# mmsyan/GoPairingBasedCryptography

Measured on AMD Instinct MI355X. Metric: BN254 pairings/s at batch 2^20 per GPU (+ G1/G2 scalar-mults/s at the same batch in roofline.scalar_mul), higher is better.
Workload: dtype int64; 1 GPU; configs[1]: batch of 1048576 independent bn254.Pair on random (G1,G2) points per GPU; batch_per_gpu=1048576

## Files before the change

### gopairingbasedcryptography_amd/csrc/bn254_constants29.hip.hpp

```cpp
#ifndef GPBC_BN254_CONSTANTS29_HIP_HPP
#define GPBC_BN254_CONSTANTS29_HIP_HPP
#define F29_P {0x187cfd47, 0x010460b6, 0x1c72a34f, 0x02d522d0, 0x1585d978, 0x02db40c0, 0x00a6e141, 0x0e5c2634, 0x0030644e}
#define F29_PINV 0x04866389
#define F29_ONE {0x157ccc21, 0x141c2758, 0x185230d3, 0x014c0419, 0x0aa36fb9, 0x1d4240ce, 0x11d54c07, 0x052ac7a8, 0x000dc836}
#define F29_TO_INTERNAL {0x13349ca1, 0x1a5d84a8, 0x0a3e5cac, 0x100249e0, 0x12b951e8, 0x0e92d304, 0x14cb95b3, 0x041b9d3d, 0x00058003}
#define F29_FROM_INTERNAL {0x058f0d9d, 0x1aea1c6e, 0x11c2cf74, 0x11d651eb, 0x1462c0a7, 0x11b7bc3c, 0x1cbd99ba, 0x183340fb, 0x000e0a77}
#define F29_B_G2 {{0x0b489658, 0x00cfd255, 0x0fdb9a77, 0x02ce89f7, 0x0033a0d4, 0x1a768545, 0x06ee3ddc, 0x106a7dc1, 0x0019316b}, {0x1b9fece0, 0x07ecccd1, 0x1069f1c7, 0x0cdf64f3, 0x0154cbe1, 0x0dd22ac0, 0x06eba4e8, 0x1929a235, 0x00283739}}
#define F29_ISO_T2 {0x130d623a, 0x0ea9efb1, 0x0fb12793, 0x1bf1335a, 0x150f3208, 0x004ff90c, 0x1b07aa3d, 0x1ae371b9, 0x001ff864}
#define F29_ISO_T3 {0x1af1f8a3, 0x00cd9858, 0x1dce6a34, 0x142e620a, 0x1bc0c667, 0x0ae94d20, 0x0db9310b, 0x12572b72, 0x000405e6}
#define F29_ISO_KFIX {0x0629460e, 0x19d018e1, 0x128d20c1, 0x106197be, 0x1858c34e, 0x0e37413a, 0x1c8aaa40, 0x058dc596, 0x0003f1e8}
#define F29_B_G1 {0x00766463, 0x1c54760a, 0x08f6927a, 0x03e40c4d, 0x1fea4f2b, 0x17c6c26a, 0x157fe417, 0x0f8056f9, 0x002958a2}
#define F29_PLAIN_TO_INTERNAL {0x059bac10, 0x0d1503a3, 0x018016b8, 0x10ab0ca8, 0x02632639, 0x02c0169f, 0x169bfd53, 0x11869d4c, 0x002a11a6}
#define F29_PLAIN_ONE {0x00000001, 0x00000000, 0x00000000, 0x00000000, 0x00000000, 0x00000000, 0x00000000, 0x00000000, 0x00000000}
#define F29_HALF_P {0x0c3e7ea3, 0x1082305b, 0x0e3951a7, 0x016a9168, 0x0ac2ecbc, 0x116da060, 0x005370a0, 0x072e131a, 0x00183227}
#define F29_EXP_SQRT {0x161f3f52, 0x1841182d, 0x071ca8d3, 0x00b548b4, 0x0561765e, 0x08b6d030, 0x0029b850, 0x1397098d, 0x000c1913}
#define F29_EXP_P34 {0x161f3f51, 0x1841182d, 0x071ca8d3, 0x00b548b4, 0x0561765e, 0x08b6d030, 0x0029b850, 0x1397098d, 0x000c1913}
#define F29_EXP_P12 {0x0c3e7ea3, 0x1082305b, 0x0e3951a7, 0x016a9168, 0x0ac2ecbc, 0x116da060, 0x005370a0, 0x072e131a, 0x00183227}
#define SVDW_G1_Z {0x157ccc21, 0x141c2758, 0x185230d3, 0x014c0419, 0x0aa36fb9, 0x1d4240ce, 0x11d54c07, 0x052ac7a8, 0x000dc836}
#define SVDW_G1_C1 {0x1d76333d, 0x0f6c3cab, 0x04d61fff, 0x025aed96, 0x1507e56c, 0x122dc278, 0x06ae4ede, 0x064ef86e, 0x0006bc8a}
#define SVDW_G1_C2 {0x01801893, 0x16741caf, 0x1210393d, 0x10c48f5b, 0x057134df, 0x12cc7ff9, 0x1768ca9c, 0x0498af45, 0x00114e0c}
#define SVDW_G1_C3 {0x1b4a814f, 0x1d686287, 0x16a42cba, 0x0bac1e79, 0x013fb16c, 0x1d850693, 0x1eba05b6, 0x0c9dae1e, 0x001b5818}
#define SVDW_G1_C4 {0x068a0e4b, 0x171eba7c, 0x0b55234f, 0x150690b3, 0x0ed0a792, 0x1ff392ca, 0x026922c2, 0x109d85a1, 0x002768eb}
#define SVDW_G2_Z {{0x157ccc21, 0x141c2758, 0x185230d3, 0x014c0419, 0x0aa36fb9, 0x1d4240ce, 0x11d54c07, 0x052ac7a8, 0x000dc836}, {0x00000000, 0x00000000, 0x00000000, 0x00000000, 0x00000000, 0x00000000, 0x00000000, 0x00000000, 0x00000000}}
#define SVDW_G2_C1 {{0x00c56279, 0x14ebf9ae, 0x082dcb4a, 0x041a8e11, 0x0ad7108d, 0x17b8c613, 0x18c389e4, 0x15954569, 0x0026f9a1}, {0x1b9fece0, 0x07ecccd1, 0x1069f1c7, 0x0cdf64f3, 0x0154cbe1, 0x0dd22ac0, 0x06eba4e8, 0x1929a235, 0x00283739}}
#define SVDW_G2_C2 {{0x01801893, 0x16741caf, 0x1210393d, 0x10c48f5b, 0x057134df, 0x12cc7ff9, 0x1768ca9c, 0x0498af45, 0x00114e0c}, {0x00000000, 0x00000000, 0x00000000, 0x00000000, 0x00000000, 0x00000000, 0x00000000, 0x00000000, 0x00000000}}
#define SVDW_G2_C3 {{0x1ac12654, 0x18b51d52, 0x02b71328, 0x0f302745, 0x18dae6df, 0x1ec740f3, 0x0ad8391f, 0x1e701b16, 0x002bf9c5}, {0x1b8c55e3, 0x07029597, 0x09a398b3, 0x06a5295f, 0x152a0cd2, 0x1080d518, 0x1295607f, 0x1129d51a, 0x00151beb}}
#define SVDW_G2_C4 {{0x1a9d7742, 0x1b78c9da, 0x18a8378f, 0x1586dd8a, 0x1c979cde, 0x1b6acebc, 0x159e5ffb, 0x15469a85, 0x002cd11a}, {0x017a140e, 0x0ccd05ab, 0x0dad5994, 0x148069b2, 0x09454dc3, 0x089e4881, 0x1813914c, 0x05d61ecb, 0x002b29a5}}
#define F29_KP_ROWS { \
{50510080, 463423804, 224178423, 182267676, 438732777, 79642451, 421445353, 64605178, -811880051, 0, 0, 0}, \
{461354567, 480487922, 164582470, 229790189, 262955361, 127565844, 432381994, 305525294, -808708645, 0, 0, 0}, \
{335328142, 497552041, 104986517, 277312702, 87177945, 175489237, 443318635, 9574498, -805537238, 0, 0, 0}, \
{209301717, 514616160, 45390564, 324835215, 448271441, 223412629, 454255276, 250494614, -802365832, 0, 0, 0}, \
{83275292, 531680279, 522665523, 372357727, 272494025, 271336022, 465191917, 491414730, -799194426, 0, 0, 0}, \
{494119779, 11873485, 463069571, 419880240, 96716609, 319259415, 476128558, 195463934, -796023019, 0, 0, 0}, \
{368093354, 28937604, 403473618, 467402753, 457810105, 367182807, 487065199, 436384050, -792851613, 0, 0, 0}, \
{242066929, 46001723, 343877665, 514925266, 282032689, 415106200, 498001840, 140433254, -789680206, 0, 0, 0}, \
{116040504, 63065842, 284281712, 25576867, 106255274, 463029593, 508938481, 381353370, -786508800, 0, 0, 0}, \
{526884991, 80129960, 224685759, 73099380, 467348770, 510952985, 519875122, 85402574, -783337393, 0, 0, 0}, \
{400858566, 97194079, 165089806, 120621893, 291571354, 22005466, 530811764, 326322690, -780165987, 0, 0, 0}, \
{274832141, 114258198, 105493853, 168144406, 115793938, 69928859, 4877493, 30371895, -776994580, 0, 0, 0}, \
{148805716, 131322317, 45897900, 215666919, 476887434, 117852251, 15814134, 271292011, -773823174, 0, 0, 0}, \
{22779291, 148386436, 523172859, 263189431, 301110018, 165775644, 26750775, 512212127, -770651768, 0, 0, 0}, \
{433623778, 165450554, 463576906, 310711944, 125332602, 213699037, 37687416, 216261331, -767480361, 0, 0, 0}, \
// ... 545 lines not shown
```

### gopairingbasedcryptography_amd/csrc/gpbc_pairing.hip

```cpp
#include "gpbc_common.hpp"
#include "wide29.hip.hpp"
#include "pairing29.hip.hpp"
#include "pairing29_pair.hip.hpp"

static_assert(LINE_BYTES_PER_PAIR == (size_t)MILLER_LINES * LINE_WORDS * sizeof(int32_t), "lines workspace row size");

__device__ __forceinline__ void line_store(int32_t *__restrict__ buf, size_t stride, size_t lane, int step, const LineS &l) {
    int32_t *b = buf + (size_t)step * LINE_WORDS * stride + lane;
    const Fe *fe[6] = {&l.c0.a0, &l.c0.a1, &l.c3.a0, &l.c3.a1, &l.c4.a0, &l.c4.a1};
#pragma unroll
    for (int e = 0; e < 6; e++)
#pragma unroll
        for (int i = 0; i < NL; i++) b[(size_t)(e * NL + i) * stride] = fe[e]->v[i];
}
__device__ __forceinline__ LineS line_load(const int32_t *__restrict__ buf, size_t stride, size_t lane, int step) {
    const int32_t *b = buf + (size_t)step * LINE_WORDS * stride + lane;
    LineS l;
    Fe *fe[6] = {&l.c0.a0, &l.c0.a1, &l.c3.a0, &l.c3.a1, &l.c4.a0, &l.c4.a1};
#pragma unroll
    for (int e = 0; e < 6; e++)
#pragma unroll
        for (int i = 0; i < NL; i++) fe[e]->v[i] = b[(size_t)(e * NL + i) * stride];
    return l;
}

__shared__ int32_t g_line_stage[27][BLOCK];
__device__ __forceinline__ void line_request(const int32_t *__restrict__ buf, size_t stride, size_t lane, int step, bool odd) {
    const int32_t *b = buf + ((size_t)step * LINE_WORDS + (odd ? 27 : 0)) * stride + lane;
#pragma unroll
    for (int r = 0; r < 27; r++) __builtin_amdgcn_global_load_lds(b + (size_t)r * stride, &g_line_stage[r][0], 4, 0, 0);
}
__device__ __forceinline__ LineS line_from_stage() {
    __builtin_amdgcn_s_waitcnt(0x0F70);
    const unsigned e = threadIdx.x & ~1u;
    LineS l;
    Fe *fe[6] = {&l.c0.a0, &l.c0.a1, &l.c3.a0, &l.c3.a1, &l.c4.a0, &l.c4.a1};
#pragma unroll
    for (int w = 0; w < LINE_WORDS; w++) fe[w / NL]->v[w % NL] = g_line_stage[w < 27 ? w : w - 27][e + (w < 27 ? 0 : 1)];
    __builtin_amdgcn_s_waitcnt(0xC07F);
    return l;
}

GPBC_KERNEL k_miller_lines(const uint8_t *__restrict__ P, const uint8_t *__restrict__ Q, int32_t *__restrict__ lines, size_t n, size_t stride) {
    size_t i = (size_t)blockIdx.x * BLOCK + threadIdx.x;
    if (i >= n) return;
    const uint8_t *p = P + i * GPBC_G1_BYTES, *q = Q + i * GPBC_G2_BYTES;
    if (g1_bytes_inf(p) || g2_bytes_inf(q)) return;
    G1A a{fe_load(p), fe_load(p + 32)};
    G2A b{f2_load(q), f2_load(q + 64)};
    int step = 0;
    miller_lines(a, b, [&](const LineS &l) { line_store(lines, stride, i, step++, l); });
}

GPBC_KERNEL k_miller_accumulate(const uint8_t *__restrict__ P, const uint8_t *__restrict__ Q, const int32_t *__restrict__ lines,
                                uint8_t *__restrict__ f_out, size_t n, size_t stride) {
    size_t lane = (size_t)blockIdx.x * BLOCK + threadIdx.x;
    size_t i = lane >> 1;
    if (i >= n) return;
    PairDpp x{(bool)(lane & 1)};
    const uint8_t *p = P + i * GPBC_G1_BYTES, *q = Q + i * GPBC_G2_BYTES;
    F6 h;
    if (g1_bytes_inf(p) || g2_bytes_inf(q)) h = f12p_one(x);
    else {
        int step = 0;
        line_request(lines, stride, i, 0, x.odd);
        h = miller_accumulate_pair(x, [&]() -> LineS {
            LineS l = line_from_stage();
            if (++step < MILLER_LINES) line_request(lines, stride, i, step, x.odd);
            return l;
        });
    }
    f6_store(f_out + i * GPBC_GT_BYTES + (x.odd ? 192 : 0), h);
}

constexpr size_t PIPELINED_MAX_PAIRS = 16384;
constexpr uint32_t PIPELINED_SPIN_LIMIT = 1u << 22;
GPBC_KERNEL k_miller_pipelined(const uint8_t *__restrict__ P, const uint8_t *__restrict__ Q, int32_t *lines, uint32_t *progress,
                               uint8_t *__restrict__ f_out, size_t n, size_t stride, unsigned n_line_blocks, uint32_t spin_limit) {
    if (blockIdx.x < n_line_blocks) {
        size_t i = (size_t)blockIdx.x * BLOCK + threadIdx.x;
        if (i >= n) return;
        const uint8_t *p = P + i * GPBC_G1_BYTES, *q = Q + i * GPBC_G2_BYTES;
        if (g1_bytes_inf(p) || g2_bytes_inf(q)) return;
        G1A a{fe_load(p), fe_load(p + 32)};
        G2A b{f2_load(q), f2_load(q + 64)};
        int step = 0;
        miller_lines(a, b, [&](const LineS &l) {
            line_store(lines, stride, i, step++, l);
            __hip_atomic_store(progress + i, (uint32_t)step, __ATOMIC_RELEASE, __HIP_MEMORY_SCOPE_AGENT);
        });
        return;
    }
    size_t lane = (size_t)(blockIdx.x - n_line_blocks) * BLOCK + threadIdx.x;
    size_t i = lane >> 1;
    if (i >= n) return;
    PairDpp x{(bool)(lane & 1)};
    const uint8_t *p = P + i * GPBC_G1_BYTES, *q = Q + i * GPBC_G2_BYTES;
    F6 h;
    if (g1_bytes_inf(p) || g2_bytes_inf(q)) h = f12p_one(x);
    else {
        int step = 0;
        bool own_lines = false;
        h = miller_accumulate_pair(x, [&]() -> LineS {
            if (!own_lines) {
                uint32_t spins = 0;
                while (__hip_atomic_load(progress + i, __ATOMIC_ACQUIRE, __HIP_MEMORY_SCOPE_AGENT) <= (uint32_t)step) {
                    __builtin_amdgcn_s_sleep(16);
                    if (++spins > spin_limit) { own_lines = true; break; }
                }
                if (own_lines) {
                    G1A a{fe_load(p), fe_load(p + 32)};
                    G2A b{f2_load(q), f2_load(q + 64)};
                    int s2 = 0;
                    miller_lines(a, b, [&](const LineS &l) { line_store(lines, stride, i, s2++, l); });
                    __threadfence();
                }
            }
            return line_load(lines, stride, i, step++);
        });
    }
    f6_store(f_out + i * GPBC_GT_BYTES + (x.odd ? 192 : 0), h);
}

constexpr int MULTI_CHUNK = 8;
constexpr size_t MULTI_GROUP = 65536;
GPBC_KERNEL k_miller_lines_chunks(const uint8_t *__restrict__ P, const uint8_t *__restrict__ Q, int32_t *__restrict__ lines,
                                  const uint64_t *__restrict__ chunk_off, size_t n_chunks, size_t n_slots, uint64_t *__restrict__ seen_lines) {
    size_t t = (size_t)blockIdx.x * BLOCK + threadIdx.x;
    if (t >= n_slots) return;
    const size_t i = t / n_chunks, c = t % n_chunks;
    const uint64_t c_lo = chunk_off[c], c_hi = chunk_off[c + 1];
    if (i == 0) { seen_lines[2 * c] = c_lo; seen_lines[2 * c + 1] = c_hi; }
    const uint64_t pair = c_lo + i;
    if (pair >= c_hi) return;
    const uint8_t *p = P + pair * GPBC_G1_BYTES, *q = Q + pair * GPBC_G2_BYTES;
    if (g1_bytes_inf(p) || g2_bytes_inf(q)) return;
    G1A a{fe_load(p), fe_load(p + 32)};
    G2A b{f2_load(q), f2_load(q + 64)};
    int step = 0;
    miller_lines(a, b, [&](const LineS &l) { line_store(lines, n_slots, t, step++, l); });
}
GPBC_KERNEL k_miller_accumulate_chunks(const uint8_t *__restrict__ P, const uint8_t *__restrict__ Q, const int32_t *__restrict__ lines,
                                       const uint64_t *__restrict__ chunk_off, uint8_t *__restrict__ f_out, size_t n_chunks, size_t n_slots,
                                       const uint64_t *__restrict__ seen_lines, uint64_t *__restrict__ seen) {
    size_t lane = (size_t)blockIdx.x * BLOCK + threadIdx.x;
    size_t c = lane >> 1;
    if (c >= n_chunks) return;
// ... 14 lines not shown
}

constexpr int FIXED_Q_CHUNK = 64;
GPBC_KERNEL k_q_lines(const uint8_t *__restrict__ Q, int32_t *__restrict__ qlines, size_t m) {
    size_t i = (size_t)blockIdx.x * BLOCK + threadIdx.x;
    if (i >= m) return;
    const uint8_t *q = Q + i * GPBC_G2_BYTES;
    if (g2_bytes_inf(q)) return;
    G2A b{f2_load(q), f2_load(q + 64)};
    int step = 0;
    miller_lines_raw(b, [&](const LineE &l) { line_store(qlines, m, i, step++, LineS{l.r0, l.r1, l.r2}); });
}
constexpr int LINE34_WORDS = 4 * NL;
GPBC_KERNEL k_q_lines_scale(const int32_t *__restrict__ qlines, int32_t *__restrict__ q34, size_t m) {
    size_t t = (size_t)blockIdx.x * BLOCK + threadIdx.x;
    if (t >= m * MILLER_LINES) return;
    const size_t i = t % m;
    const int li = (int)(t / m);
    LineS r = line_load(qlines, m, i, li);
    F2 inv = f2_inv(f2_norm(r.c0));
    F2 c3 = f2_mul(f2_norm(r.c3), inv), c4 = f2_mul(f2_norm(r.c4), inv);
    int32_t *o = q34 + (size_t)li * LINE34_WORDS * m + i;
    const Fe *fe[4] = {&c3.a0, &c3.a1, &c4.a0, &c4.a1};
#pragma unroll
    for (int e = 0; e < 4; e++)
#pragma unroll
        for (int w = 0; w < NL; w++) o[(size_t)(e * NL + w) * m] = fe[e]->v[w];
}
constexpr int LINE_POINT_GROUP = 8;
GPBC_KERNEL_G1 k_g1_line_point(const uint8_t *__restrict__ P, int32_t *__restrict__ out, size_t n) {
    const size_t base = ((size_t)blockIdx.x * BLOCK + threadIdx.x) * LINE_POINT_GROUP;
    if (base >= n) return;
    const int cnt = n - base < (size_t)LINE_POINT_GROUP ? (int)(n - base) : LINE_POINT_GROUP;
    fe_batch_inverse<LINE_POINT_GROUP>(cnt, [&](int j) { return fe_load(P + (base + j) * GPBC_G1_BYTES + 32); }, [&](int j, const Fe &yinv) {
        const uint8_t *pb = P + (base + j) * GPBC_G1_BYTES;
        Fe xoy = fe_mul(fe_load(pb), yinv);
        int32_t *o = out + (base + j) * 20;
#pragma unroll
        for (int w = 0; w < NL; w++) { o[w] = xoy.v[w]; o[NL + w] = yinv.v[w]; }
        o[18] = g1_bytes_inf(pb) ? 1 : 0;
        o[19] = 0;
    });
}
GPBC_KERNEL k_miller_accumulate_fixed_q(const int32_t *__restrict__ Pint, const uint8_t *__restrict__ Q, const int32_t *__restrict__ q34,
                                        uint8_t *__restrict__ f_out, size_t m, size_t k, size_t L, size_t n_c) {
    size_t lane = (size_t)blockIdx.x * BLOCK + threadIdx.x;
    size_t t = lane >> 1;
    if (t >= n_c * k) return;
    PairDpp x{(bool)(lane & 1)};
    const size_t c = t / k, j = t % k;
    const size_t lo = c * L, hi = (c + 1) * L < m ? (c + 1) * L : m;
    int vi[FIXED_Q_CHUNK], n = 0;
    for (size_t i = lo; i < hi; i++)
        if (!Pint[(j * m + i) * 20 + 18] && !g2_bytes_inf(Q + i * GPBC_G2_BYTES)) vi[n++] = (int)i;
    F6 h;
    if (n == 0) h = f12p_one(x);
    else h = miller_accumulate_multi_34(x, n, [&](int p, int li) -> Line34 {
        const size_t i = (size_t)vi[p];
        const int32_t *lb = q34 + ((size_t)li * LINE34_WORDS + (x.odd ? 2 * NL : 0)) * m + i;
        const int32_t *pp = Pint + (j * m + i) * 20 + (x.odd ? NL : 0);
        F2 coef;
        Fe pc;
#pragma unroll
        for (int w = 0; w < NL; w++) { coef.a0.v[w] = lb[(size_t)w * m]; coef.a1.v[w] = lb[(size_t)(NL + w) * m]; pc.v[w] = pp[w]; }
        const F2 mine = f2_mul_fe(coef, pc), other = x.swap(mine);
        return Line34{f2_sel(x.odd, other, mine), f2_sel(x.odd, mine, other)};
    });
    f6_store(f_out + (j * n_c + c) * GPBC_GT_BYTES + (x.odd ? 192 : 0), h);
// ... 752 lines not shown
```

### gopairingbasedcryptography_amd/csrc/pairing29.hip.hpp

```cpp
#ifndef GPBC_PAIRING29_HIP_HPP
#define GPBC_PAIRING29_HIP_HPP
#include "bn254_constants.hip.hpp"
#include "tower29.hip.hpp"

namespace gpbc {

struct G1A { Fe x, y; };
struct G2A { F2 x, y; };
struct G2P { F2 x, y, z; };
struct LineE { F2 r0, r1, r2; };

GPBC_INLINE int ate_naf_digit(int i) { constexpr int8_t D[BN254_ATE_NAF_LEN] = BN254_ATE_NAF; return D[i]; }

GPBC_INLINE F2 f2_mul_9mi_n(const F2 &x) {
    return F2{fe_reduce_arith_norm(fe_add(fe_add(fe_mul8_norm(x.a0), x.a0), x.a1)), fe_reduce_arith_norm(fe_sub(fe_add(fe_mul8_norm(x.a1), x.a1), x.a0))};
}
template <bool ISO = false> GPBC_INLINE void g2_double_step(G2P &t, LineE &l) {
    F2 A = f2_halve(f2_mul(t.x, t.y));
    F2 B = f2_sqr(t.y);
    F2 C = f2_sqr(t.z);
    F2 C3 = f2_norm(f2_add(f2_dbl(C), C));
    F2 E = ISO ? f2_mul_9mi_n(C3) : f2_mul(C3, b_twist29());
    F2 F = f2_add(f2_dbl(E), E);
    F2 G = ISO ? f2_add(E, f2_halve(f2_norm(f2_add(B, E)))) : f2_halve(f2_norm(f2_add(B, F)));
// ... 7 lines not shown
    l.r1 = f2_norm(f2_add(f2_dbl(J), J));
    l.r2 = f2_sub(E, B);
}
GPBC_INLINE void g2_add_step(G2P &t, LineE &l, const G2A &q) {
    F2 O = f2_sub(t.y, f2_mul(q.y, t.z));
    F2 L = f2_sub(t.x, f2_mul(q.x, t.z));
    F2 C = f2_sqr(O);
    F2 D = f2_sqr(L);
    F2 E = f2_mul(L, D);
    F2 F = f2_mul(t.z, C);
    F2 G = f2_mul(t.x, D);
    F2 H = f2_norm(f2_sub(f2_add(E, F), f2_dbl(G)));
    F2 t1 = f2_mul(t.y, E);
    t.x = f2_mul(L, H);
    t.y = f2_norm(f2_sub(f2_mul(f2_sub(G, H), O), t1));
    t.z = f2_mul(E, t.z);
    l.r0 = L;
    l.r1 = f2_neg(O);
    l.r2 = f2_sub(f2_mul(q.x, O), f2_mul(L, q.y));
}
GPBC_INLINE void g2_line_step(const G2P &t, LineE &l, const G2A &q) {
    F2 O = f2_sub(t.y, f2_mul(q.y, t.z));
    F2 L = f2_sub(t.x, f2_mul(q.x, t.z));
    l.r0 = L;
    l.r1 = f2_neg(O);
    l.r2 = f2_sub(f2_mul(q.x, O), f2_mul(L, q.y));
}
struct LineS { F2 c0, c3, c4; };
constexpr int MILLER_LINES = 88;
constexpr int LINE_WORDS = 6 * NL;

GPBC_INLINE LineS line_scale(const LineE &l, const G1A &p) { return LineS{f2_mul_fe(l.r0, p.y), f2_mul_fe(l.r1, p.x), l.r2}; }

template <class Sink> GPBC_INLINE void miller_lines(const G1A &p0, const G2A &q0, Sink &&sink) {
    constexpr int32_t T2[NL] = F29_ISO_T2, T3[NL] = F29_ISO_T3, KF[NL] = F29_ISO_KFIX;
    const Fe t2 = fe_const(T2), t3 = fe_const(T3);
    const G1A p{fe_mul(p0.x, t2), fe_mul(p0.y, t3)};
    const G2A q{f2_mul_fe(q0.x, t2), f2_mul_fe(q0.y, t3)};
    G2P t{q.x, q.y, f2_one()};
    const F2 ny = f2_neg(q.y);
    LineE l;
    for (int i = BN254_ATE_NAF_LEN - 2; i >= 0; i--) {
        g2_double_step<true>(t, l);
        sink(line_scale(l, p));
        int d = ate_naf_digit(i);
        if (d != 0) {
            g2_add_step(t, l, G2A{q.x, f2_sel(d > 0, q.y, ny)});
            sink(line_scale(l, p));
        }
    }
    G2A q1{f2_mul(f2_conj(q.x), gamma29(1, 2)), f2_mul(f2_conj(q.y), gamma29(1, 3))};
    G2A q2{f2_mul(q.x, gamma29(2, 2)), f2_neg(f2_mul(q.y, gamma29(2, 3)))};
    g2_add_step(t, l, q1);
    sink(line_scale(l, p));
    g2_line_step(t, l, q2);
    const Fe k = fe_const(KF);
    sink(LineS{f2_mul_fe(l.r0, fe_mul(p.y, k)), f2_mul_fe(l.r1, fe_mul(p.x, k)), f2_mul_fe(l.r2, k)});
}

template <class Sink> GPBC_INLINE void miller_lines_raw(const G2A &q, Sink &&sink) {
    G2P t{q.x, q.y, f2_one()};
    const F2 ny = f2_neg(q.y);
    LineE l;
    for (int i = BN254_ATE_NAF_LEN - 2; i >= 0; i--) {
        g2_double_step(t, l);
        sink(l);
        int d = ate_naf_digit(i);
        if (d != 0) {
            g2_add_step(t, l, G2A{q.x, f2_sel(d > 0, q.y, ny)});
            sink(l);
        }
    }
    G2A q1{f2_mul(f2_conj(q.x), gamma29(1, 2)), f2_mul(f2_conj(q.y), gamma29(1, 3))};
    G2A q2{f2_mul(q.x, gamma29(2, 2)), f2_neg(f2_mul(q.y, gamma29(2, 3)))};
    g2_add_step(t, l, q1);
    sink(l);
    g2_line_step(t, l, q2);
    sink(l);
}

template <int G, class LoadY, class Emit> GPBC_INLINE void fe_batch_inverse(int cnt, LoadY &&y_at, Emit &&emit) {
    Fe y[G], pre[G];
#pragma unroll
    for (int j = 0; j < G; j++) {
        y[j] = fe_one();
        if (j < cnt) {
            Fe v = y_at(j);
            if (!fe_is_zero(v)) y[j] = v;
        }
// ... 117 lines not shown
```

### gopairingbasedcryptography_amd/csrc/pairing29_pair.hip.hpp

```cpp
#ifndef GPBC_PAIRING29_PAIR_HIP_HPP
#define GPBC_PAIRING29_PAIR_HIP_HPP
#include "pairing29.hip.hpp"
#include "tower29_pair.hip.hpp"

namespace gpbc {

template <class X, class Src> GPBC_INLINE F6 miller_accumulate_pair(const X &x, Src &&next) {
    LineS l0 = next();
    F6 h = f6_norm(f6_sel(x.odd, F6{l0.c3, l0.c4, f2_zero()}, F6{l0.c0, f2_zero(), f2_zero()}));
    for (int i = BN254_ATE_NAF_LEN - 2; i >= 0; i--) {
        if (i != BN254_ATE_NAF_LEN - 2) {
            h = f12p_sqr<true>(x, h);
            LineS l = next();
            h = f12p_mul_034<true>(x, h, l.c0, l.c3, l.c4);
        }
        if (ate_naf_digit(i) != 0) {
            LineS l = next();
            h = f12p_mul_034<true>(x, h, l.c0, l.c3, l.c4);
        }
    }
    for (int k = 0; k < 2; k++) {
        LineS l = next();
        h = f12p_mul_034<true>(x, h, l.c0, l.c3, l.c4);
    }
    return h;
}

template <class X, class LineAt> GPBC_INLINE F6 miller_accumulate_multi(const X &x, int m, LineAt &&line) {
    int li = 0;
    auto mul_lines = [&](F6 h, int from) {
        int p = from;
        for (; p + 1 < m; p += 2) {
            LineS a = line(p, li), b = line(p + 1, li);
            h = f12p_mul(x, h, f12p_mul_034_by_034(x, a.c0, a.c3, a.c4, b.c0, b.c3, b.c4));
        }
        if (p < m) { LineS l = line(p, li); h = f12p_mul_034(x, h, l.c0, l.c3, l.c4); }
        li++;
        return h;
    };
    LineS l0 = line(0, li);
    F6 h = f6_sel(x.odd, F6{l0.c3, l0.c4, f2_zero()}, F6{l0.c0, f2_zero(), f2_zero()});
    h = mul_lines(h, 1);
    for (int i = BN254_ATE_NAF_LEN - 2; i >= 0; i--) {
        if (i != BN254_ATE_NAF_LEN - 2) {
            h = f12p_sqr(x, h);
            if (m >= 2) h = f6_reduce_arith(h);
            h = mul_lines(h, 0);
        }
        if (ate_naf_digit(i) != 0) h = mul_lines(h, 0);
    }
    for (int k = 0; k < 2; k++) h = mul_lines(h, 0);
    return h;
}

struct Line34 { F2 c3, c4; };
template <class X, class LineAt> GPBC_INLINE F6 miller_accumulate_multi_34(const X &x, int m, LineAt &&line) {
    int li = 0;
    auto mul_lines = [&](F6 h, int from) {
        for (int p = from; p < m; p++) { Line34 l = line(p, li); h = f12p_mul_34<true>(x, h, l.c3, l.c4); }
        li++;
        return h;
    };
    Line34 l0 = line(0, li);
    F6 h = f6_norm(f6_sel(x.odd, F6{l0.c3, l0.c4, f2_zero()}, F6{f2_one(), f2_zero(), f2_zero()}));
    h = mul_lines(h, 1);
    for (int i = BN254_ATE_NAF_LEN - 2; i >= 0; i--) {
        if (i != BN254_ATE_NAF_LEN - 2) h = mul_lines(f12p_sqr<true>(x, h), 0);
        if (ate_naf_digit(i) != 0) h = mul_lines(h, 0);
    }
    for (int k = 0; k < 2; k++) h = mul_lines(h, 0);
    return h;
}

template <class X> GPBC_NOINLINE void f12p_expt_to(const X &x, F6 &z, const F6 &b) {
    constexpr int8_t D[GPBC_U_CHAIN_LEN] = GPBC_U_CHAIN;
    F6 tab[3];
    bool flipped = false;
    F6 r = f12p_cyclo_sqr<true>(x, b);
    tab[0] = f6_norm(f12p_mul(x, f6_norm(b), r));
#pragma unroll 1
    for (int k = 1; k < 3; k++) {
        r = f12p_cyclo_sqr_run(x, tab[k - 1], 2, flipped);
        tab[k] = f6_norm(f12p_mul<true>(x, r, tab[k - 1]));
    }
    r = tab[u_chain_entry(D[GPBC_U_CHAIN_LEN - 1])];
    int run = 0;
    for (int i = GPBC_U_CHAIN_LEN - 2; i >= 0; i--) {
        run++;
        int d = D[i];
        if (d != 0) {
            r = f12p_cyclo_sqr_run(x, r, run, flipped);
            run = 0;
            F6 t = tab[u_chain_entry(d)];
            if ((d < 0) != flipped) t = f6_norm(f12p_conj(x, t));
            r = f12p_mul<true>(x, r, t);
        }
    }
// ... 90 lines not shown
```

### gopairingbasedcryptography_amd/csrc/tower29.hip.hpp

```cpp
#ifndef GPBC_TOWER29_HIP_HPP
#define GPBC_TOWER29_HIP_HPP
#include "fe29.hip.hpp"

namespace gpbc {

struct F2 { Fe a0, a1; };
struct F6 { F2 b0, b1, b2; };
struct F12 { F6 c0, c1; };

GPBC_INLINE F2 f2_zero() { return F2{fe_zero(), fe_zero()}; }
GPBC_INLINE F2 f2_one() { return F2{fe_one(), fe_zero()}; }
GPBC_INLINE F2 f2_add(const F2 &x, const F2 &y) { return F2{fe_add(x.a0, y.a0), fe_add(x.a1, y.a1)}; }
GPBC_INLINE F2 f2_sub(const F2 &x, const F2 &y) { return F2{fe_sub(x.a0, y.a0), fe_sub(x.a1, y.a1)}; }
GPBC_INLINE F2 f2_dbl(const F2 &x) { return F2{fe_dbl(x.a0), fe_dbl(x.a1)}; }
GPBC_INLINE F2 f2_neg(const F2 &x) { return F2{fe_neg(x.a0), fe_neg(x.a1)}; }
GPBC_INLINE F2 f2_conj(const F2 &x) { return F2{x.a0, fe_neg(x.a1)}; }
GPBC_INLINE F2 f2_norm(const F2 &x) { return F2{fe_norm(x.a0), fe_norm(x.a1)}; }
GPBC_INLINE F2 f2_reduce(const F2 &x) { return F2{fe_reduce(x.a0), fe_reduce(x.a1)}; }
GPBC_INLINE F2 f2_halve(const F2 &x) { return F2{fe_halve(x.a0), fe_halve(x.a1)}; }
GPBC_INLINE bool f2_is_zero(const F2 &x) { return fe_is_zero(x.a0) && fe_is_zero(x.a1); }

GPBC_INLINE Fe fe_sel(bool c, const Fe &a, const Fe &b) {
    Fe r;
#pragma unroll
// ... 134 lines not shown
    F2 m12 = f2_mul(f2_sub(x.b1, x.b2), f2_sub(y.b1, y.b2));
    F2 m01 = f2_mul(f2_sub(x.b0, x.b1), f2_sub(y.b0, y.b1));
    F2 m02 = f2_mul(f2_sub(x.b0, x.b2), f2_sub(y.b0, y.b2));
    F2 c0 = f2_add(f2_mul_xi_t<RX>(f2_norm(f2_sub(f2_add(t1, t2), m12))), t0);
    F2 c1 = f2_add(f2_sub(f2_add(t0, t1), m01), f2_mul_xi_t<RX>(t2));
    F2 c2 = f2_add(f2_sub(f2_add(t0, t2), m02), t1);
    return F6{f2_norm(c0), f2_norm(c1), f2_norm(c2)};
}
GPBC_INLINE F6 f6_sqr(const F6 &x) {
    F2 s0 = f2_sqr(x.b0);
    F2 m01 = f2_mul(x.b0, x.b1);
    F2 s2 = f2_sqr_n(f2_add(f2_sub(x.b0, x.b1), x.b2));
    F2 m12 = f2_mul(x.b1, x.b2);
    F2 s4 = f2_sqr(x.b2);
    F2 c0 = f2_add(s0, f2_mul_xi_n(f2_norm(f2_dbl(m12))));
    F2 c1 = f2_add(f2_dbl(m01), f2_mul_xi_n(s4));
    F2 c2 = f2_add(f2_norm(f2_dbl(f2_add(m01, m12))), f2_sub(f2_sub(s2, s0), s4));
    return F6{c0, f2_norm(c1), f2_norm(c2)};
}
GPBC_INLINE F6 f6_mul_f2(const F6 &x, const F2 &k) { return F6{f2_mul(x.b0, k), f2_mul(x.b1, k), f2_mul(x.b2, k)}; }
template <bool RX, bool NORM01 = true> GPBC_INLINE F6 f6_mul_01_t(const F6 &x, const F2 &c0, const F2 &c1, const F2 &s01) {
    F2 a = f2_mul(x.b0, c0), b = f2_mul(x.b1, c1);
    F2 t0 = f2_add(f2_mul_xi_t<RX>(f2_sub(f2_mul(f2_norm(f2_add(x.b1, x.b2)), c1), b)), a);
    F2 t1 = f2_sub(f2_sub(f2_mul(f2_norm(f2_add(x.b0, x.b1)), s01), a), b);
    F2 t2 = f2_add(f2_sub(f2_mul(f2_norm(f2_add(x.b0, x.b2)), c0), a), b);
    return F6{NORM01 ? f2_norm(t0) : t0, t1, f2_norm(t2)};
}
GPBC_INLINE F6 f6_mul_01(const F6 &x, const F2 &c0, const F2 &c1, const F2 &s01) { return f6_mul_01_t<true>(x, c0, c1, s01); }
template <bool RX> GPBC_INLINE F6 f6_mul_01_pn_t(const F6 &x, const F2 &c0, const F2 &c1, const F2 &d01) {
    F2 a = f2_mul(x.b0, c0), b = f2_mul(x.b1, c1);
    F2 t0 = f2_add(f2_mul_xi_t<RX>(f2_sub(b, f2_mul(f2_sub(x.b1, x.b2), c1))), a);
    F2 t1 = f2_sub(f2_add(a, b), f2_mul(f2_sub(x.b0, x.b1), d01));
    F2 t2 = f2_add(f2_sub(a, f2_mul(f2_sub(x.b0, x.b2), c0)), b);
    return F6{t0, t1, f2_norm(t2)};
}
GPBC_INLINE F6 f6_inv(const F6 &x) {
    F2 t0 = f2_norm(f2_sub(f2_sqr(x.b0), f2_mul_xi_n(f2_mul(x.b1, x.b2))));
    F2 t1 = f2_norm(f2_sub(f2_mul_xi_n(f2_sqr(x.b2)), f2_mul(x.b0, x.b1)));
    F2 t2 = f2_sub(f2_sqr(x.b1), f2_mul(x.b0, x.b2));
    F2 inner = f2_norm(f2_add(f2_mul(x.b2, t1), f2_mul(x.b1, t2)));
    F2 d = f2_norm(f2_add(f2_mul(x.b0, t0), f2_mul_xi_n(inner)));
    d = f2_inv(d);
    return F6{f2_mul(t0, d), f2_mul(t1, d), f2_mul(t2, d)};
}

GPBC_INLINE F12 f12_one() { return F12{F6{f2_one(), f2_zero(), f2_zero()}, F6{f2_zero(), f2_zero(), f2_zero()}}; }
GPBC_INLINE F12 f12_conj(const F12 &x) { return F12{x.c0, f6_neg(x.c1)}; }
GPBC_INLINE F12 f12_mul(const F12 &x, const F12 &y) {
    F6 t0 = f6_mul(x.c0, y.c0), t1 = f6_mul(x.c1, y.c1);
    F6 m = f6_mul(f6_norm(f6_add(x.c0, x.c1)), f6_norm(f6_add(y.c0, y.c1)));
    F6 c1 = f6_sub(f6_sub(m, t0), t1);
    F6 c0 = f6_add(t0, f6_mul_v(t1));
    return F12{f6_reduce(f6_norm(c0)), f6_reduce(f6_norm(c1))};
}
GPBC_INLINE F12 f12_sqr(const F12 &x) {
    F6 m = f6_mul(x.c0, x.c1);
    F6 s = f6_norm(f6_add(x.c0, x.c1));
    F6 t = f6_norm(f6_add(x.c0, f6_mul_v(x.c1)));
    F6 st = f6_mul(s, t);
    F6 mv = f6_mul_v(m);
    return F12{f6_norm(f6_sub(f6_sub(st, m), mv)), f6_norm(f6_add(m, m))};
}
GPBC_INLINE F12 f12_inv(const F12 &x) {
    F6 t1 = f6_mul_v(f6_sqr(x.c1));
    F6 d = f6_inv(f6_norm(f6_sub(f6_sqr(x.c0), t1)));
    return F12{f6_mul(x.c0, d), f6_neg(f6_mul(x.c1, d))};
// ... 69 lines not shown
```

### gopairingbasedcryptography_amd/csrc/tower29_pair.hip.hpp

```cpp
#ifndef GPBC_TOWER29_PAIR_HIP_HPP
#define GPBC_TOWER29_PAIR_HIP_HPP
#include "tower29.hip.hpp"

namespace gpbc {

GPBC_INLINE F6 f6_sel(bool c, const F6 &a, const F6 &b) { return F6{f2_sel(c, a.b0, b.b0), f2_sel(c, a.b1, b.b1), f2_sel(c, a.b2, b.b2)}; }
GPBC_INLINE F6 f6_dbl(const F6 &x) { return f6_add(x, x); }

#if defined(__HIPCC__) && !defined(GPBC_BOUNDS)
struct PairDpp {
    bool odd;
    __device__ __forceinline__ static int32_t sw(int32_t v) {
#if defined(__HIP_DEVICE_COMPILE__)
        return __builtin_amdgcn_mov_dpp(v, 0xB1, 0xF, 0xF, true);
#else
        return v;
#endif
    }
    __device__ __forceinline__ Fe swap(const Fe &a) const {
        Fe r;
#pragma unroll
        for (int i = 0; i < NL; i++) r.v[i] = sw(a.v[i]);
        return r;
    }
// ... 32 lines not shown
template <class X> GPBC_INLINE F6 f6p_add_partner(const X &x, const F6 &a) {
    return F6{f2_add(a.b0, x.swap(a.b0)), f2_add(a.b1, x.swap(a.b1)), f2_add(a.b2, x.swap(a.b2))};
}

template <class X> GPBC_INLINE F6 f12p_one(const X &x) { return f6_sel(x.odd, F6{f2_zero(), f2_zero(), f2_zero()}, F6{f2_one(), f2_zero(), f2_zero()}); }
template <class X> GPBC_INLINE F6 f12p_conj(const X &x, const F6 &h) { return f6_sel(x.odd, f6_neg(h), h); }

template <bool PN = false, class X> GPBC_INLINE F6 f12p_sqr(const X &x, const F6 &h) {
    F6 p = x.swap(h);
    F6 s = f6_norm(f6_add(h, p));
    F6 t = f6_norm(f6_add(p, f6_mul_v_t<false>(h)));
    F6 r = PN ? f6_mul_pn_t<false>(f6_sel(x.odd, s, h), f6_sel(x.odd, t, p)) : f6_mul_t<false>(f6_sel(x.odd, s, h), f6_sel(x.odd, t, p));
    F6 pr = x.swap(r);
    F6 even_out = f6_sub(f6_sub(pr, r), f6_mul_v_t<false>(r));
    F6 odd_out = f6_dbl(pr);
    return f6_norm(f6_sel(x.odd, odd_out, even_out));
}

template <bool PN = false, class X> GPBC_INLINE F6 f12p_mul_034(const X &x, const F6 &h, const F2 &c0, const F2 &c3, const F2 &c4) {
    F2 s34 = f2_norm(PN ? f2_sub(c3, c4) : f2_add(c3, c4));
    F6 r0 = f6_mul_f2(h, c0);
    F6 r1 = PN ? f6_mul_01_pn_t<false>(h, c3, c4, s34) : f6_mul_01_t<false, false>(h, c3, c4, s34);
    F6 send = f6_sel(x.odd, f6_mul_v_t<false>(r1), r1);
    F6 sum = f6p_add_swap(x, r0, send);
    return PN ? f6_reduce_arith_norm(sum) : f6_reduce_arith(f6_norm(sum));
}

template <bool PN = false, class X> GPBC_INLINE F6 f12p_mul_34(const X &x, const F6 &h, const F2 &c3, const F2 &c4) {
    F2 s34 = f2_norm(PN ? f2_sub(c3, c4) : f2_add(c3, c4));
    F6 r1 = PN ? f6_mul_01_pn_t<false>(h, c3, c4, s34) : f6_mul_01_t<false, false>(h, c3, c4, s34);
    F6 send = f6_sel(x.odd, f6_mul_v_t<false>(r1), r1);
    F6 sum = f6p_add_swap(x, h, send);
    return PN ? f6_reduce_arith_norm(sum) : f6_reduce_arith(f6_norm(sum));
}

template <class X> GPBC_INLINE F6 f12p_mul_034_by_034(const X &x, const F2 &c0, const F2 &c3, const F2 &c4, const F2 &d0, const F2 &d3, const F2 &d4) {
    F2 x1 = f2_sel(x.odd, c4, c0), y1 = f2_sel(x.odd, d4, d0);
    F2 x2 = f2_sel(x.odd, f2_norm(f2_add(c0, c3)), c3), y2 = f2_sel(x.odd, f2_norm(f2_add(d0, d3)), d3);
    F2 x3 = f2_norm(f2_add(f2_sel(x.odd, c0, c3), c4)), y3 = f2_norm(f2_add(f2_sel(x.odd, d0, d3), d4));
    F6 mine{f2_mul(x1, y1), f2_mul(x2, y2), f2_mul(x3, y3)};
    F6 other = x.swap(mine);
    F2 t = f2_sub(f2_sub(mine.b2, other.b0), f2_sel(x.odd, mine.b0, mine.b1));
    F2 u = f2_sel(x.odd, f2_sub(f2_sub(mine.b1, other.b0), other.b1), f2_add(mine.b0, f2_mul_xi(other.b0)));
    return f6_reduce_arith(f6_norm(F6{u, f2_sel(x.odd, t, mine.b1), f2_sel(x.odd, f2_zero(), t)}));
}

#if defined(__HIP_DEVICE_COMPILE__) && !defined(GPBC_BOUNDS)
__shared__ i32x4 g_f6_park[14][64];
struct F6Park {
    GPBC_INLINE explicit F6Park(const F6 &v) {
        const Fe *fe[6] = {&v.b0.a0, &v.b0.a1, &v.b1.a0, &v.b1.a1, &v.b2.a0, &v.b2.a1};
        int32_t w[56];
#pragma unroll
        for (int e = 0; e < 6; e++)
#pragma unroll
            for (int i = 0; i < NL; i++) w[e * NL + i] = fe[e]->v[i];
        w[54] = 0; w[55] = 0;
        const unsigned lane = f2_arg_lane();
#pragma unroll
        for (int c = 0; c < 14; c++) g_f6_park[c][lane] = i32x4{w[4 * c], w[4 * c + 1], w[4 * c + 2], w[4 * c + 3]};
    }
    GPBC_INLINE F6 get() const {
        int32_t w[56];
        const unsigned lane = f2_arg_lane();
#pragma unroll
        for (int c = 0; c < 14; c++) { i32x4 t = g_f6_park[c][lane]; w[4 * c] = t.x; w[4 * c + 1] = t.y; w[4 * c + 2] = t.z; w[4 * c + 3] = t.w; }
// ... 123 lines not shown
```

Before: 7.568 million pairings/s.

## Pre-scale line coefficients by two to use a cheaper sparse 034 multiply

Adds an X2 variant of miller_lines that scales the G1 y-coordinate and the final fixup constant by two, so the c0 line coefficient arrives doubled. The accumulate side then uses a new f6_mul_01_pn4_t that forms (b0+b2+b1)*s and (b1-b0-b2)*d, which avoids one Karatsuba-style multiply or subtraction chain in the sparse line multiply. The 34-only multi path compensates by halving the cached line inputs. It adds extra doublings and normalisations and depends on consistent scaling across the line-generation and accumulation kernels. Pairing correctness relies on the constant-factor scaling being eliminated by the final exponentiation.

```diff
diff --git a/gopairingbasedcryptography_amd/csrc/bn254_constants29.hip.hpp b/gopairingbasedcryptography_amd/csrc/bn254_constants29.hip.hpp
--- a/gopairingbasedcryptography_amd/csrc/bn254_constants29.hip.hpp
+++ b/gopairingbasedcryptography_amd/csrc/bn254_constants29.hip.hpp
@@ -9,6 +9,8 @@
 #define F29_ISO_T2 {0x130d623a, 0x0ea9efb1, 0x0fb12793, 0x1bf1335a, 0x150f3208, 0x004ff90c, 0x1b07aa3d, 0x1ae371b9, 0x001ff864}
 #define F29_ISO_T3 {0x1af1f8a3, 0x00cd9858, 0x1dce6a34, 0x142e620a, 0x1bc0c667, 0x0ae94d20, 0x0db9310b, 0x12572b72, 0x000405e6}
 #define F29_ISO_KFIX {0x0629460e, 0x19d018e1, 0x128d20c1, 0x106197be, 0x1858c34e, 0x0e37413a, 0x1c8aaa40, 0x058dc596, 0x0003f1e8}
+#define F29_ISO_T3_X2 {0x15e3f146, 0x019b30b1, 0x1b9cd468, 0x085cc415, 0x17818ccf, 0x15d29a41, 0x1b726216, 0x04ae56e4, 0x00080bcd}
+#define F29_ISO_KFIX_X2 {0x0f060e62, 0x100dad14, 0x1da99f82, 0x13c8c6db, 0x160237fb, 0x180371dc, 0x19d59101, 0x1ae5e61d, 0x00244443}
 #define F29_B_G1 {0x00766463, 0x1c54760a, 0x08f6927a, 0x03e40c4d, 0x1fea4f2b, 0x17c6c26a, 0x157fe417, 0x0f8056f9, 0x002958a2}
 #define F29_PLAIN_TO_INTERNAL {0x059bac10, 0x0d1503a3, 0x018016b8, 0x10ab0ca8, 0x02632639, 0x02c0169f, 0x169bfd53, 0x11869d4c, 0x002a11a6}
 #define F29_PLAIN_ONE {0x00000001, 0x00000000, 0x00000000, 0x00000000, 0x00000000, 0x00000000, 0x00000000, 0x00000000, 0x00000000}
diff --git a/gopairingbasedcryptography_amd/csrc/gpbc_pairing.hip b/gopairingbasedcryptography_amd/csrc/gpbc_pairing.hip
--- a/gopairingbasedcryptography_amd/csrc/gpbc_pairing.hip
+++ b/gopairingbasedcryptography_amd/csrc/gpbc_pairing.hip
@@ -49,7 +49,7 @@
     G1A a{fe_load(p), fe_load(p + 32)};
     G2A b{f2_load(q), f2_load(q + 64)};
     int step = 0;
-    miller_lines(a, b, [&](const LineS &l) { line_store(lines, stride, i, step++, l); });
+    miller_lines<true>(a, b, [&](const LineS &l) { line_store(lines, stride, i, step++, l); });
 }
 
 GPBC_KERNEL k_miller_accumulate(const uint8_t *__restrict__ P, const uint8_t *__restrict__ Q, const int32_t *__restrict__ lines,
@@ -85,7 +85,7 @@
         G1A a{fe_load(p), fe_load(p + 32)};
         G2A b{f2_load(q), f2_load(q + 64)};
         int step = 0;
-        miller_lines(a, b, [&](const LineS &l) {
+        miller_lines<true>(a, b, [&](const LineS &l) {
             line_store(lines, stride, i, step++, l);
             __hip_atomic_store(progress + i, (uint32_t)step, __ATOMIC_RELEASE, __HIP_MEMORY_SCOPE_AGENT);
         });
@@ -112,7 +112,7 @@
                     G1A a{fe_load(p), fe_load(p + 32)};
                     G2A b{f2_load(q), f2_load(q + 64)};
                     int s2 = 0;
-                    miller_lines(a, b, [&](const LineS &l) { line_store(lines, stride, i, s2++, l); });
+                    miller_lines<true>(a, b, [&](const LineS &l) { line_store(lines, stride, i, s2++, l); });
                     __threadfence();
                 }
             }
@@ -193,8 +193,9 @@
     const size_t base = ((size_t)blockIdx.x * BLOCK + threadIdx.x) * LINE_POINT_GROUP;
     if (base >= n) return;
     const int cnt = n - base < (size_t)LINE_POINT_GROUP ? (int)(n - base) : LINE_POINT_GROUP;
-    fe_batch_inverse<LINE_POINT_GROUP>(cnt, [&](int j) { return fe_load(P + (base + j) * GPBC_G1_BYTES + 32); }, [&](int j, const Fe &yinv) {
+    fe_batch_inverse<LINE_POINT_GROUP>(cnt, [&](int j) { return fe_load(P + (base + j) * GPBC_G1_BYTES + 32); }, [&](int j, const Fe &y_inverse) {
         const uint8_t *pb = P + (base + j) * GPBC_G1_BYTES;
+        const Fe yinv = fe_halve(y_inverse);
         Fe xoy = fe_mul(fe_load(pb), yinv);
         int32_t *o = out + (base + j) * 20;
 #pragma unroll
diff --git a/gopairingbasedcryptography_amd/csrc/pairing29.hip.hpp b/gopairingbasedcryptography_amd/csrc/pairing29.hip.hpp
--- a/gopairingbasedcryptography_amd/csrc/pairing29.hip.hpp
+++ b/gopairingbasedcryptography_amd/csrc/pairing29.hip.hpp
@@ -63,10 +63,10 @@
 
 GPBC_INLINE LineS line_scale(const LineE &l, const G1A &p) { return LineS{f2_mul_fe(l.r0, p.y), f2_mul_fe(l.r1, p.x), l.r2}; }
 
-template <class Sink> GPBC_INLINE void miller_lines(const G1A &p0, const G2A &q0, Sink &&sink) {
-    constexpr int32_t T2[NL] = F29_ISO_T2, T3[NL] = F29_ISO_T3, KF[NL] = F29_ISO_KFIX;
+template <bool X2 = false, class Sink> GPBC_INLINE void miller_lines(const G1A &p0, const G2A &q0, Sink &&sink) {
+    constexpr int32_t T2[NL] = F29_ISO_T2, T3[NL] = F29_ISO_T3, KF[NL] = F29_ISO_KFIX, T3X2[NL] = F29_ISO_T3_X2, KFX2[NL] = F29_ISO_KFIX_X2;
     const Fe t2 = fe_const(T2), t3 = fe_const(T3);
-    const G1A p{fe_mul(p0.x, t2), fe_mul(p0.y, t3)};
+    const G1A p{fe_mul(p0.x, t2), fe_mul(p0.y, fe_const(X2 ? T3X2 : T3))};
     const G2A q{f2_mul_fe(q0.x, t2), f2_mul_fe(q0.y, t3)};
     G2P t{q.x, q.y, f2_one()};
     const F2 ny = f2_neg(q.y);
@@ -85,7 +85,7 @@
     g2_add_step(t, l, q1);
     sink(line_scale(l, p));
     g2_line_step(t, l, q2);
-    const Fe k = fe_const(KF);
+    const Fe k = fe_const(X2 ? KFX2 : KF);
     sink(LineS{f2_mul_fe(l.r0, fe_mul(p.y, k)), f2_mul_fe(l.r1, fe_mul(p.x, k)), f2_mul_fe(l.r2, k)});
 }
 
diff --git a/gopairingbasedcryptography_amd/csrc/pairing29_pair.hip.hpp b/gopairingbasedcryptography_amd/csrc/pairing29_pair.hip.hpp
--- a/gopairingbasedcryptography_amd/csrc/pairing29_pair.hip.hpp
+++ b/gopairingbasedcryptography_amd/csrc/pairing29_pair.hip.hpp
@@ -7,21 +7,21 @@
 
 template <class X, class Src> GPBC_INLINE F6 miller_accumulate_pair(const X &x, Src &&next) {
     LineS l0 = next();
-    F6 h = f6_norm(f6_sel(x.odd, F6{l0.c3, l0.c4, f2_zero()}, F6{l0.c0, f2_zero(), f2_zero()}));
+    F6 h = f6_norm(f6_sel(x.odd, F6{f2_dbl(l0.c3), f2_dbl(l0.c4), f2_zero()}, F6{l0.c0, f2_zero(), f2_zero()}));
     for (int i = BN254_ATE_NAF_LEN - 2; i >= 0; i--) {
         if (i != BN254_ATE_NAF_LEN - 2) {
             h = f12p_sqr<true>(x, h);
             LineS l = next();
-            h = f12p_mul_034<true>(x, h, l.c0, l.c3, l.c4);
+            h = f12p_mul_034_x2(x, h, l.c0, l.c3, l.c4);
         }
         if (ate_naf_digit(i) != 0) {
             LineS l = next();
-            h = f12p_mul_034<true>(x, h, l.c0, l.c3, l.c4);
+            h = f12p_mul_034_x2(x, h, l.c0, l.c3, l.c4);
         }
     }
     for (int k = 0; k < 2; k++) {
         LineS l = next();
-        h = f12p_mul_034<true>(x, h, l.c0, l.c3, l.c4);
+        h = f12p_mul_034_x2(x, h, l.c0, l.c3, l.c4);
     }
     return h;
 }
@@ -57,12 +57,12 @@
 template <class X, class LineAt> GPBC_INLINE F6 miller_accumulate_multi_34(const X &x, int m, LineAt &&line) {
     int li = 0;
     auto mul_lines = [&](F6 h, int from) {
-        for (int p = from; p < m; p++) { Line34 l = line(p, li); h = f12p_mul_34<true>(x, h, l.c3, l.c4); }
+        for (int p = from; p < m; p++) { Line34 l = line(p, li); h = f12p_mul_34_half(x, h, l.c3, l.c4); }
         li++;
         return h;
     };
     Line34 l0 = line(0, li);
-    F6 h = f6_norm(f6_sel(x.odd, F6{l0.c3, l0.c4, f2_zero()}, F6{f2_one(), f2_zero(), f2_zero()}));
+    F6 h = f6_norm(f6_sel(x.odd, F6{f2_dbl(l0.c3), f2_dbl(l0.c4), f2_zero()}, F6{f2_one(), f2_zero(), f2_zero()}));
     h = mul_lines(h, 1);
     for (int i = BN254_ATE_NAF_LEN - 2; i >= 0; i--) {
         if (i != BN254_ATE_NAF_LEN - 2) h = mul_lines(f12p_sqr<true>(x, h), 0);
diff --git a/gopairingbasedcryptography_amd/csrc/tower29.hip.hpp b/gopairingbasedcryptography_amd/csrc/tower29.hip.hpp
--- a/gopairingbasedcryptography_amd/csrc/tower29.hip.hpp
+++ b/gopairingbasedcryptography_amd/csrc/tower29.hip.hpp
@@ -190,6 +190,15 @@
     F2 t0 = f2_add(f2_mul_xi_t<RX>(f2_sub(b, f2_mul(f2_sub(x.b1, x.b2), c1))), a);
     F2 t1 = f2_sub(f2_add(a, b), f2_mul(f2_sub(x.b0, x.b1), d01));
     F2 t2 = f2_add(f2_sub(a, f2_mul(f2_sub(x.b0, x.b2), c0)), b);
+    return F6{t0, t1, f2_norm(t2)};
+}
+template <bool X2> GPBC_INLINE F6 f6_mul_01_pn4_t(const F6 &x, const F2 &c0, const F2 &c1, const F2 &s, const F2 &d) {
+    F2 e = f2_add(x.b0, x.b2);
+    F2 A = f2_mul(x.b0, c0), B = f2_mul(x.b2, c1);
+    F2 C = f2_mul(f2_norm(f2_add(e, x.b1)), s), Dn = f2_mul(f2_norm(f2_sub(x.b1, e)), d);
+    F2 t0 = X2 ? f2_dbl(f2_norm(f2_add(f2_mul_xi(B), A))) : f2_add(f2_mul_xi_nn(B), A);
+    F2 t1 = f2_sub(f2_add(C, Dn), X2 ? f2_dbl(B) : B);
+    F2 t2 = f2_sub(f2_sub(C, Dn), X2 ? f2_dbl(A) : A);
     return F6{t0, t1, f2_norm(t2)};
 }
 GPBC_INLINE F6 f6_inv(const F6 &x) {
diff --git a/gopairingbasedcryptography_amd/csrc/tower29_pair.hip.hpp b/gopairingbasedcryptography_amd/csrc/tower29_pair.hip.hpp
--- a/gopairingbasedcryptography_amd/csrc/tower29_pair.hip.hpp
+++ b/gopairingbasedcryptography_amd/csrc/tower29_pair.hip.hpp
@@ -88,6 +88,18 @@
     F6 send = f6_sel(x.odd, f6_mul_v_t<false>(r1), r1);
     F6 sum = f6p_add_swap(x, h, send);
     return PN ? f6_reduce_arith_norm(sum) : f6_reduce_arith(f6_norm(sum));
+}
+
+template <class X> GPBC_INLINE F6 f12p_mul_034_x2(const X &x, const F6 &h, const F2 &c0x2, const F2 &c3, const F2 &c4) {
+    F6 r0 = f6_mul_f2(h, c0x2);
+    F6 r1 = f6_mul_01_pn4_t<true>(h, c3, c4, f2_norm(f2_add(c3, c4)), f2_norm(f2_sub(c3, c4)));
+    F6 send = f6_sel(x.odd, f6_mul_v_t<false>(r1), r1);
+    return f6_reduce_arith_norm(f6p_add_swap(x, r0, send));
+}
+template <class X> GPBC_INLINE F6 f12p_mul_34_half(const X &x, const F6 &h, const F2 &c3h, const F2 &c4h) {
+    F6 r1 = f6_mul_01_pn4_t<false>(h, f2_norm(f2_dbl(c3h)), f2_norm(f2_dbl(c4h)), f2_norm(f2_add(c3h, c4h)), f2_norm(f2_sub(c3h, c4h)));
+    F6 send = f6_sel(x.odd, f6_mul_v_t<false>(r1), r1);
+    return f6_reduce_arith_norm(f6p_add_swap(x, h, send));
 }
 
 template <class X> GPBC_INLINE F6 f12p_mul_034_by_034(const X &x, const F2 &c0, const F2 &c3, const F2 &c4, const F2 &d0, const F2 &d3, const F2 &d4) {
```

New measurement: 7.773 million pairings/s, median of 6. 1.03x the previous value.
